# elfi-dev/elfi

Hardware: NVIDIA H100
Metric: accepted particles/sec (higher is better)
Workload: dtype f64

## Files before the change

### elfi_b200/csrc/common.cuh

```cuda
#pragma once

#include <cuda.h>
#include <cuda_runtime.h>

#include <cstdarg>
#include <cstdint>
#include <cstdio>
#include <cstring>

#include "../../include/elfi_b200.h"

namespace elfi {

void set_error(const char* fmt, ...);

#define ELFI_CUDA_OK(expr)                                                              \
    do {                                                                                \
        cudaError_t _e = (expr);                                                        \
        if (_e != cudaSuccess) {                                                        \
            ::elfi::set_error("%s failed: %s (%s:%d)", #expr, cudaGetErrorString(_e),   \
                              __FILE__, __LINE__);                                      \
            cudaGetLastError();       \
            return ELFI_B200_ERR_CUDA;                                                  \
        }                                                                               \
    } while (0)

#define ELFI_REQUIRE(cond, ...)                                                         \
    do {                                                                                \
        if (!(cond)) {                                                                  \
            ::elfi::set_error(__VA_ARGS__);                                             \
            return ELFI_B200_ERR_ARG;                                                   \
        }                                                                               \
    } while (0)

typedef CUresult (*tensor_map_encode_fn)(CUtensorMap*, CUtensorMapDataType, cuuint32_t, void*,
                                         const cuuint64_t*, const cuuint64_t*,
                                         const cuuint32_t*, const cuuint32_t*,
                                         CUtensorMapInterleave, CUtensorMapSwizzle,
                                         CUtensorMapL2promotion, CUtensorMapFloatOOBfill);

}

struct elfi_b200_ctx {
    int device;
    int sm_count;
    size_t smem_optin;
    elfi::tensor_map_encode_fn encode_tiled;
    void* scratch;
    size_t scratch_bytes;
    void* pinned;
    size_t pinned_bytes;
    void* dev_stage;
    size_t dev_stage_bytes;
    cudaStream_t copy_stream[2];
    cudaEvent_t copy_event[4];
};

namespace elfi {

void* ctx_scratch(elfi_b200_ctx* ctx, size_t bytes);

int make_rowmajor_f64_map(elfi_b200_ctx* ctx, const double* base, int64_t rows, int64_t cols,
                          int64_t ld, int box_rows, CUtensorMap* out);

inline bool tma_compatible(const void* base, int64_t ld) {
    return (reinterpret_cast<uintptr_t>(base) % 16 == 0) && ((ld * 8) % 16 == 0);
}

__device__ __forceinline__ uint32_t smem_u32(const void* p) {
    return static_cast<uint32_t>(__cvta_generic_to_shared(p));
}

__device__ __forceinline__ void mbar_init(uint32_t bar, uint32_t count) {
    asm volatile("mbarrier.init.shared::cta.b64 [%0], %1;" ::"r"(bar), "r"(count) : "memory");
}

__device__ __forceinline__ void mbar_fence_init() {
    asm volatile("fence.mbarrier_init.release.cluster;" ::: "memory");
    asm volatile("fence.proxy.async.shared::cta;" ::: "memory");
}

__device__ __forceinline__ void mbar_arrive_expect_tx(uint32_t bar, uint32_t bytes) {
    asm volatile("mbarrier.arrive.expect_tx.shared::cta.b64 _, [%0], %1;" ::"r"(bar), "r"(bytes)
                 : "memory");
}

__device__ __forceinline__ bool mbar_try_wait(uint32_t bar, uint32_t parity) {
    uint32_t ok;
    asm volatile(
        "{\n"
        ".reg .pred p;\n"
        "mbarrier.try_wait.parity.shared::cta.b64 p, [%1], %2;\n"
        "selp.u32 %0, 1, 0, p;\n"
// ... 35 lines not shown
```

### elfi_b200/csrc/ctx.cu

```cuda
#include "common.cuh"

namespace elfi {

static thread_local char g_error[512] = "";

void set_error(const char* fmt, ...) {
    va_list ap;
    va_start(ap, fmt);
    vsnprintf(g_error, sizeof(g_error), fmt, ap);
    va_end(ap);
}

void* ctx_scratch(elfi_b200_ctx* ctx, size_t bytes) {
    if (bytes <= ctx->scratch_bytes) return ctx->scratch;
    size_t want = bytes + (bytes >> 2) + (1u << 20);
    want = (want + 255) & ~size_t(255);
    if (ctx->scratch) {
        if (cudaDeviceSynchronize() != cudaSuccess || cudaFree(ctx->scratch) != cudaSuccess) {
            set_error("scratch release failed: %s", cudaGetErrorString(cudaGetLastError()));
            ctx->scratch = nullptr;
            ctx->scratch_bytes = 0;
            return nullptr;
        }
        ctx->scratch = nullptr;
        ctx->scratch_bytes = 0;
    }
    void* p = nullptr;
    cudaError_t e = cudaMalloc(&p, want);
    if (e != cudaSuccess) {
        set_error("cudaMalloc(%zu) for scratch failed: %s", want, cudaGetErrorString(e));
        cudaGetLastError();
        return nullptr;
    }
    ctx->scratch = p;
    ctx->scratch_bytes = want;
    return p;
}

int make_rowmajor_f64_map(elfi_b200_ctx* ctx, const double* base, int64_t rows, int64_t cols,
                          int64_t ld, int box_rows, CUtensorMap* out) {
    ELFI_REQUIRE(ctx->encode_tiled != nullptr, "cuTensorMapEncodeTiled entry point unavailable");
    ELFI_REQUIRE(tma_compatible(base, ld), "matrix is not TMA compatible (16-byte base/stride)");
    cuuint64_t dims[2] = {static_cast<cuuint64_t>(cols), static_cast<cuuint64_t>(rows)};
    cuuint64_t strides[1] = {static_cast<cuuint64_t>(ld) * sizeof(double)};
    cuuint32_t box[2] = {16u, static_cast<cuuint32_t>(box_rows)};
    cuuint32_t estr[2] = {1u, 1u};
    CUresult r = ctx->encode_tiled(out, CU_TENSOR_MAP_DATA_TYPE_FLOAT64, 2,
                                   const_cast<double*>(base), dims, strides, box, estr,
                                   CU_TENSOR_MAP_INTERLEAVE_NONE, CU_TENSOR_MAP_SWIZZLE_128B,
                                   CU_TENSOR_MAP_L2_PROMOTION_L2_256B,
                                   CU_TENSOR_MAP_FLOAT_OOB_FILL_NONE);
    if (r != CUDA_SUCCESS) {
        set_error("cuTensorMapEncodeTiled failed with CUresult %d (rows=%lld cols=%lld ld=%lld)",
                  static_cast<int>(r), (long long)rows, (long long)cols, (long long)ld);
        return ELFI_B200_ERR_CUDA;
    }
    return ELFI_B200_OK;
}

}

extern "C" {

int elfi_b200_version(void) { return ELFI_B200_VERSION; }

const char* elfi_b200_last_error(void) { return elfi::g_error; }

int elfi_b200_ctx_create(int device, elfi_b200_ctx** out) {
    ELFI_REQUIRE(out != nullptr, "ctx_create: out is NULL");
// ... 9 lines not shown
        elfi::set_error("ctx_create: device %d is sm_%d%d; this library is built for sm_90a only",
                        device, prop.major, prop.minor);
        return ELFI_B200_ERR_UNSUPPORTED;
    }
    elfi_b200_ctx* ctx = new elfi_b200_ctx();
    memset(ctx, 0, sizeof(*ctx));
    ctx->device = device;
    ctx->sm_count = prop.multiProcessorCount;
    ctx->smem_optin = prop.sharedMemPerBlockOptin;
    void* fn = nullptr;
    cudaDriverEntryPointQueryResult qres;
    cudaError_t e = cudaGetDriverEntryPoint("cuTensorMapEncodeTiled", &fn, cudaEnableDefault, &qres);
    if (e != cudaSuccess || qres != cudaDriverEntryPointSuccess || fn == nullptr) {
        elfi::set_error("ctx_create: cuTensorMapEncodeTiled not available from the driver");
        delete ctx;
        cudaGetLastError();
        return ELFI_B200_ERR_CUDA;
    }
    ctx->encode_tiled = reinterpret_cast<elfi::tensor_map_encode_fn>(fn);
    for (int i = 0; i < 2; ++i)
        ELFI_CUDA_OK(cudaStreamCreateWithFlags(&ctx->copy_stream[i], cudaStreamNonBlocking));
    for (int i = 0; i < 4; ++i)
        ELFI_CUDA_OK(cudaEventCreateWithFlags(&ctx->copy_event[i], cudaEventDisableTiming));
    *out = ctx;
    return ELFI_B200_OK;
}

int elfi_b200_ctx_destroy(elfi_b200_ctx* ctx) {
    if (!ctx) return ELFI_B200_OK;
    cudaSetDevice(ctx->device);
    cudaDeviceSynchronize();
    if (ctx->scratch) cudaFree(ctx->scratch);
    if (ctx->dev_stage) cudaFree(ctx->dev_stage);
    if (ctx->pinned) cudaFreeHost(ctx->pinned);
    for (int i = 0; i < 2; ++i)
        if (ctx->copy_stream[i]) cudaStreamDestroy(ctx->copy_stream[i]);
    for (int i = 0; i < 4; ++i)
        if (ctx->copy_event[i]) cudaEventDestroy(ctx->copy_event[i]);
    delete ctx;
    return ELFI_B200_OK;
}

int elfi_b200_ctx_sm_count(const elfi_b200_ctx* ctx) { return ctx ? ctx->sm_count : 0; }

int elfi_b200_allgather_particles(elfi_b200_ctx* const* ctxs, int64_t n_ctx, const double* const* send,
                                  int64_t rows, int64_t width, double* const* recv,
                                  void* const* streams) {
    ELFI_REQUIRE(ctxs && send && recv && streams && n_ctx >= 1 && n_ctx <= 64,
                 "allgather_particles: bad argument");
    ELFI_REQUIRE(rows >= 0 && width >= 1, "allgather_particles: bad shape");
    for (int64_t g = 0; g < n_ctx; ++g)
        ELFI_REQUIRE(ctxs[g] && (rows == 0 || (send[g] && recv[g])), "allgather_particles: NULL entry %lld",
                     (long long)g);
    if (rows == 0) return ELFI_B200_OK;
    const size_t bytes = size_t(rows) * size_t(width) * 8;
    int caller_device = 0;
    ELFI_CUDA_OK(cudaGetDevice(&caller_device));
    struct Restore {
        int d;
        ~Restore() { cudaSetDevice(d); }
    } restore{caller_device};
    for (int64_t d = 0; d < n_ctx; ++d) {
        ELFI_CUDA_OK(cudaSetDevice(ctxs[d]->device));
        for (int64_t s = 0; s < n_ctx; ++s) {
            if (ctxs[s]->device == ctxs[d]->device) continue;
            int can = 0;
// ... 34 lines not shown
```

### elfi_b200/csrc/distance.cu

```cuda
#include <cstdlib>

#include "rowstream.cuh"

extern "C" int elfi_b200_colmoments_f64(elfi_b200_ctx* ctx, const double* S, int64_t ldS, int64_t B,
                                        int64_t D, double* out, void* stream);

namespace elfi {

struct DistParams {
    const double* obs;
    const double* W;
    double* d_out;
    uint32_t* mask;
    int K;
    int has_thr;
    const double* shift_src;
    double* mom_partial;
    const double* thr_dev;
    double thr[ELFI_B200_MAX_NESTED];
    __device__ __forceinline__ double threshold(int k) const {
        return thr_dev ? __ldg(thr_dev + k) : thr[k];
    }
};

__device__ __forceinline__ void dist_setup_shared(uint8_t* aux, const DistParams& p, int D,
                                                  bool weighted) {
    const int Dp = ((D + RS_BOX_COLS - 1) / RS_BOX_COLS) * RS_BOX_COLS;
    double* obs_s = reinterpret_cast<double*>(aux);
    for (int j = threadIdx.x; j < Dp; j += blockDim.x) obs_s[j] = j < D ? p.obs[j] : 0.0;
    if (weighted) {
        double* w_s = obs_s + Dp;
        for (int k = 0; k < p.K; ++k)
            for (int j = threadIdx.x; j < Dp; j += blockDim.x)
                w_s[size_t(k) * Dp + j] = j < D ? p.W[size_t(k) * D + j] : 0.0;
// ... 273 lines not shown
dist_direct_kernel(const double* __restrict__ S, int64_t ld, int64_t B, int D, DistParams p) {
    const int64_t row = int64_t(blockIdx.x) * blockDim.x + threadIdx.x;
    const int lane = threadIdx.x & 31;
    const int K = p.K;
    bool ok = row < B;
    if (ok) {
        const double* r = S + row * ld;
        for (int k = 0; k < K; ++k) {
            double acc = 0.0;
            if (p.W != nullptr) {
                const double* w = p.W + size_t(k) * D;
                for (int j = 0; j < D; ++j) {
                    const double d = __dsub_rn(__ldg(r + j), __ldg(p.obs + j));
                    acc = __dadd_rn(acc, __dmul_rn(__ldg(w + j), __dmul_rn(d, d)));
                }
            } else {
                for (int j = 0; j < D; ++j) {
                    const double d = __dsub_rn(__ldg(r + j), __ldg(p.obs + j));
                    acc = __dadd_rn(acc, __dmul_rn(d, d));
                }
            }
            const double dist = sqrt(acc);
            p.d_out[row * K + k] = dist;
            if (p.has_thr) ok = ok && (dist <= p.threshold(k));
        }
    }
    if (p.mask != nullptr) {
        const uint32_t bits = __ballot_sync(0xffffffffu, ok && p.has_thr);
        if (lane == 0 && (row - lane) < B) p.mask[row >> 5] = bits;
    }
}

__global__ void __launch_bounds__(1024)
compact_mask_kernel(const uint32_t* __restrict__ mask, int64_t nwords, int64_t B,
                    int32_t* __restrict__ idx, int64_t* __restrict__ n_out) {
    __shared__ int64_t warp_sums[32];
    __shared__ int64_t base_s;
    const int tid = threadIdx.x;
    const int lane = tid & 31;
    const int wid = tid >> 5;
    const int64_t first = int64_t(blockIdx.x) * 1024;

    int64_t before = 0;
    for (int64_t w = tid; w < first; w += 1024) before += __popc(mask[w]);
    for (int o = 16; o > 0; o >>= 1) before += __shfl_xor_sync(0xffffffffu, before, o);
    if (lane == 0) warp_sums[wid] = before;
    __syncthreads();
    if (tid == 0) {
        int64_t t = 0;
        for (int i = 0; i < 32; ++i) t += warp_sums[i];
        base_s = t;
    }
    __syncthreads();
    const int64_t base = base_s;
    __syncthreads();

    const int64_t w = first + tid;
    const uint32_t bits = w < nwords ? mask[w] : 0u;
    const int cnt = __popc(bits);
    int incl = cnt;
    for (int o = 1; o < 32; o <<= 1) {
        const int t = __shfl_up_sync(0xffffffffu, incl, o);
        if (lane >= o) incl += t;
    }
    if (lane == 31) warp_sums[wid] = incl;
    __syncthreads();
    if (wid == 0) {
        int64_t v = warp_sums[lane];
        int64_t inc2 = v;
        for (int o = 1; o < 32; o <<= 1) {
            const int64_t t = __shfl_up_sync(0xffffffffu, inc2, o);
            if (lane >= o) inc2 += t;
        }
        warp_sums[lane] = inc2 - v;
        if (lane == 31 && blockIdx.x == gridDim.x - 1 && n_out != nullptr) *n_out = base + inc2;
    }
    __syncthreads();
    int64_t pos = base + warp_sums[wid] + (incl - cnt);
    if (idx != nullptr) {
        uint32_t b = bits;
        while (b) {
            const int bit = __ffs(b) - 1;
            b &= b - 1;
            idx[pos++] = int32_t(w * 32 + bit);
        }
    }
}

int launch_compact_mask(const uint32_t* mask, int64_t B, int32_t* idx, int64_t* n_out,
                        cudaStream_t stream) {
    const int64_t nwords = (B + 31) / 32;
    if (nwords == 0) {
        if (n_out) ELFI_CUDA_OK(cudaMemsetAsync(n_out, 0, sizeof(int64_t), stream));
        return ELFI_B200_OK;
    }
    const unsigned blocks = unsigned((nwords + 1023) / 1024);
    compact_mask_kernel<<<blocks, 1024, 0, stream>>>(mask, nwords, B, idx, n_out);
    ELFI_CUDA_OK(cudaGetLastError());
    return ELFI_B200_OK;
}

int launch_dist(elfi_b200_ctx* ctx, const double* S, int64_t ldS, int64_t B, int64_t D,
                const double* obs, const double* W, int64_t K, const double* thr_host,
                double* d_out, uint32_t* mask, cudaStream_t stream,
                const double* thr_dev = nullptr) {
    DistParams p;
    memset(&p, 0, sizeof(p));
    p.obs = obs;
    p.W = W;
    p.d_out = d_out;
    p.mask = mask;
    p.K = int(K);
    p.has_thr = thr_host != nullptr || thr_dev != nullptr;
    p.thr_dev = thr_dev;
    if (thr_host)
        for (int k = 0; k < K; ++k) p.thr[k] = thr_host[k];
    if (B == 0) return ELFI_B200_OK;

    const int64_t Dp = ((D + RS_BOX_COLS - 1) / RS_BOX_COLS) * RS_BOX_COLS;
    const bool use_tma = D >= RS_BOX_COLS && tma_compatible(S, ldS);
    if (use_tma) {
        const size_t aux = size_t(Dp) * 8 * (W ? (1 + K) : 1);
        if (rs_pick_stages(ctx->smem_optin, aux) >= 2) {
            if (W == nullptr) return rowstream_launch<EuclidConsumer>(ctx, S, ldS, B, D, aux, p, stream);
            if (K == 1) return rowstream_launch<WeightedConsumer>(ctx, S, ldS, B, D, aux, p, stream);
            if (K <= 2) return rowstream_launch<NestedConsumer<2>>(ctx, S, ldS, B, D, aux, p, stream);
            if (K <= 3) return rowstream_launch<NestedConsumer<3>>(ctx, S, ldS, B, D, aux, p, stream);
            if (K <= 4) return rowstream_launch<NestedConsumer<4>>(ctx, S, ldS, B, D, aux, p, stream);
            if (K <= 5) return rowstream_launch<NestedConsumer<5>>(ctx, S, ldS, B, D, aux, p, stream);
            if (K <= 6) return rowstream_launch<NestedConsumer<6>>(ctx, S, ldS, B, D, aux, p, stream);
// ... 224 lines not shown
    MetricParams p;
    memset(&p, 0, sizeof(p));
    p.obs = obs;
    p.V = V;
    p.d_out = d_out;
    p.mask = mask;
    p.K = 1;
    p.has_thr = thr_host != nullptr;
    if (thr_host) p.thr[0] = thr_host[0];
    if (B == 0) return ELFI_B200_OK;
    const int64_t Dp = ((D + RS_BOX_COLS - 1) / RS_BOX_COLS) * RS_BOX_COLS;
    const size_t aux = size_t(Dp) * 8 * 2;
    if (D >= RS_BOX_COLS && tma_compatible(S, ldS) && rs_pick_stages(ctx->smem_optin, aux) >= 2)
        return rowstream_launch<SeuclidConsumer>(ctx, S, ldS, B, D, aux, p, stream);
    seuclid_direct_kernel<<<unsigned((B + 255) / 256), 256, 0, stream>>>(S, ldS, B, int(D), p);
    ELFI_CUDA_OK(cudaGetLastError());
    return ELFI_B200_OK;
}

static int check_dist_args(const void* S, int64_t ldS, int64_t B, int64_t D, const void* obs,
                           const void* W, int64_t K, const void* thr, const void* acc_idx) {
    ELFI_REQUIRE(B >= 0 && D >= 1, "dist: bad shape B=%lld D=%lld", (long long)B, (long long)D);
    ELFI_REQUIRE(B == 0 || S != nullptr, "dist: S is NULL");
    ELFI_REQUIRE(obs != nullptr, "dist: obs is NULL");
    ELFI_REQUIRE(ldS >= D, "dist: ldS (%lld) < D (%lld)", (long long)ldS, (long long)D);
    ELFI_REQUIRE(K >= 1 && K <= ELFI_B200_MAX_NESTED, "dist: K=%lld outside [1, %d]",
                 (long long)K, ELFI_B200_MAX_NESTED);
    ELFI_REQUIRE(W != nullptr || K == 1, "dist: K=%lld needs a weight matrix", (long long)K);
    ELFI_REQUIRE(acc_idx == nullptr || thr != nullptr, "dist: acc_idx requires thresholds");
    ELFI_REQUIRE(B < (int64_t(1) << 31), "dist: B must fit int32 row indices");
    return ELFI_B200_OK;
}

}

extern "C" {

int elfi_b200_dist_euclid_thr_f64(elfi_b200_ctx* ctx, const double* S, int64_t ldS, int64_t B,
                                  int64_t D, const double* obs, const double* W, int64_t K,
                                  const double* thr_host, double* d_out, int32_t* acc_idx,
                                  int64_t* n_acc, void* stream_) {
    using namespace elfi;
    ELFI_REQUIRE(ctx != nullptr, "dist: ctx is NULL");
    int rc = check_dist_args(S, ldS, B, D, obs, W, K, thr_host, acc_idx);
    if (rc) return rc;
    ELFI_REQUIRE(B == 0 || d_out != nullptr, "dist: d_out is NULL");
    cudaStream_t stream = static_cast<cudaStream_t>(stream_);
    ELFI_CUDA_OK(cudaSetDevice(ctx->device));
    uint32_t* mask = nullptr;
    if (thr_host != nullptr) {
        const size_t nwords = size_t((B + 31) / 32);
        mask = static_cast<uint32_t*>(ctx_scratch(ctx, nwords * 4 + 256));
        if (!mask) return ELFI_B200_ERR_NOMEM;
    }
    rc = launch_dist(ctx, S, ldS, B, D, obs, W, K, thr_host, d_out, mask, stream);
    if (rc) return rc;
    if (thr_host != nullptr && (acc_idx != nullptr || n_acc != nullptr))
        return launch_compact_mask(mask, B, acc_idx, n_acc, stream);
    return ELFI_B200_OK;
}

int elfi_b200_dist_euclid_thr_dev_f64(elfi_b200_ctx* ctx, const double* S, int64_t ldS, int64_t B,
                                      int64_t D, const double* obs, const double* W, int64_t K,
                                      const double* thr_dev, double* d_out, int32_t* acc_idx,
                                      int64_t* n_acc, void* stream_) {
    using namespace elfi;
    ELFI_REQUIRE(ctx != nullptr && thr_dev != nullptr, "dist: ctx or thr_dev is NULL");
    int rc = check_dist_args(S, ldS, B, D, obs, W, K, thr_dev, acc_idx);
    if (rc) return rc;
    ELFI_REQUIRE(B == 0 || d_out != nullptr, "dist: d_out is NULL");
    cudaStream_t stream = static_cast<cudaStream_t>(stream_);
    ELFI_CUDA_OK(cudaSetDevice(ctx->device));
    const size_t nwords = size_t((B + 31) / 32);
    uint32_t* mask = static_cast<uint32_t*>(ctx_scratch(ctx, nwords * 4 + 256));
    if (!mask) return ELFI_B200_ERR_NOMEM;
    rc = launch_dist(ctx, S, ldS, B, D, obs, W, K, nullptr, d_out, mask, stream, thr_dev);
    if (rc) return rc;
    if (acc_idx != nullptr || n_acc != nullptr)
        return launch_compact_mask(mask, B, acc_idx, n_acc, stream);
    return ELFI_B200_OK;
}

int elfi_b200_dist_euclid_mom_f64(elfi_b200_ctx* ctx, const double* S, int64_t ldS, int64_t B,
                                  int64_t D, const double* obs, const double* W, int64_t K,
                                  const double* thr_host, const double* thr_dev, double* d_out,
                                  int32_t* acc_idx, int64_t* n_acc, double* moments,
                                  void* stream_) {
    using namespace elfi;
    ELFI_REQUIRE(ctx != nullptr && moments != nullptr, "dist_mom: ctx or moments is NULL");
    ELFI_REQUIRE(!(thr_host && thr_dev), "dist_mom: give thresholds on the host OR on the device");
    const void* thr = thr_host ? static_cast<const void*>(thr_host) : thr_dev;
    int rc = check_dist_args(S, ldS, B, D, obs, W, K, thr, acc_idx);
    if (rc) return rc;
    ELFI_REQUIRE(B >= 1 && d_out != nullptr, "dist_mom: needs at least one row and d_out");
    cudaStream_t stream = static_cast<cudaStream_t>(stream_);
    ELFI_CUDA_OK(cudaSetDevice(ctx->device));
    const int64_t Dp = ((D + RS_BOX_COLS - 1) / RS_BOX_COLS) * RS_BOX_COLS;
    const size_t aux = NestedMomentsConsumer<2>::aux_bytes(Dp, K);
    const bool fused = W != nullptr && D >= RS_BOX_COLS && tma_compatible(S, ldS) &&
                       rs_pick_stages(ctx->smem_optin, aux) >= 2;
    const size_t mask_bytes = (size_t((B + 31) / 32) * 4 + 255) & ~size_t(255);
    const size_t part_bytes = fused ? size_t(ctx->sm_count) * 16 * 2 * D * 8 : 0;
    uint8_t* base = static_cast<uint8_t*>(ctx_scratch(ctx, mask_bytes + part_bytes + 256));
    if (!base) return ELFI_B200_ERR_NOMEM;
    uint32_t* mask = thr ? reinterpret_cast<uint32_t*>(base) : nullptr;
    if (!fused) {
        rc = launch_dist(ctx, S, ldS, B, D, obs, W, K, thr_host, d_out, mask, stream, thr_dev);
        if (rc) return rc;
        if (thr && (acc_idx != nullptr || n_acc != nullptr)) {
// ... 172 lines not shown
```

### elfi_b200/csrc/select.cu

```cuda
#include <cstdlib>

#include "bitonic.cuh"
#include "eqweight.h"
#include "pairwise.cuh"

namespace elfi {

constexpr int SORT_CHUNK = 1024;
constexpr int SORT_WARPS = 8;

__global__ void __launch_bounds__(256)
sort_prepare_kernel(const double* __restrict__ keys, int64_t n, uint64_t* __restrict__ ukeys,
                    int32_t* __restrict__ vals, uint32_t* __restrict__ ghist) {
    __shared__ uint32_t h[8 * 256];
    for (int i = threadIdx.x; i < 8 * 256; i += blockDim.x) h[i] = 0;
    __syncthreads();
    const int64_t stride = int64_t(gridDim.x) * blockDim.x;
    for (int64_t i = int64_t(blockIdx.x) * blockDim.x + threadIdx.x; i < n; i += stride) {
        const uint64_t u = key_to_u64(keys[i]);
        ukeys[i] = u;
        vals[i] = int32_t(i);
#pragma unroll
        for (int p = 0; p < 8; ++p) atomicAdd(&h[p * 256 + ((u >> (8 * p)) & 255)], 1u);
    }
    __syncthreads();
    for (int i = threadIdx.x; i < 8 * 256; i += blockDim.x)
        if (h[i]) atomicAdd(&ghist[i], h[i]);
}

__device__ __forceinline__ bool pass_trivial(const uint32_t* ghist, int pass, int64_t n,
                                             uint64_t first_key) {
    return ghist[pass * 256 + ((first_key >> (8 * pass)) & 255)] == uint32_t(n);
}

__global__ void __launch_bounds__(SORT_WARPS * 32)
// ... 171 lines not shown
    int32_t col0[APPEND_MAX_SRC];
    int32_t n_src, total_width;
};

__global__ void __launch_bounds__(256)
accept_append_kernel(const int32_t* __restrict__ acc_idx, const int64_t* __restrict__ n_acc,
                     AppendSources src, double* __restrict__ dst, int64_t ld_dst, int64_t capacity,
                     const int64_t* __restrict__ count) {
    const int64_t base = *count;
    int64_t room = capacity - base;
    if (room < 0) room = 0;
    const int64_t rows = *n_acc < room ? *n_acc : room;
    const int64_t total = rows * src.total_width;
    const int64_t stride = int64_t(gridDim.x) * blockDim.x;
    for (int64_t t = int64_t(blockIdx.x) * blockDim.x + threadIdx.x; t < total; t += stride) {
        const int64_t j = t / src.total_width;
        const int c = int(t - j * src.total_width);
        const int64_t row = acc_idx ? int64_t(acc_idx[j]) : j;
        int k = 0;
#pragma unroll
        for (int q = 1; q < APPEND_MAX_SRC; ++q)
            if (q < src.n_src && c >= src.col0[q]) k = q;
        dst[(base + j) * ld_dst + c] = src.ptr[k][row * src.ld[k] + (c - src.col0[k])];
    }
}

__global__ void accept_count_kernel(const int64_t* __restrict__ n_acc, int64_t capacity,
                                    int64_t* __restrict__ count, int64_t* __restrict__ dropped) {
    int64_t room = capacity - *count;
    if (room < 0) room = 0;
    const int64_t rows = *n_acc < room ? *n_acc : room;
    if (dropped) *dropped += *n_acc - rows;
    *count += rows;
}

__global__ void __launch_bounds__(256)
gather2_rows_kernel(const double* __restrict__ A, int64_t ldA, int64_t nA,
                    const double* __restrict__ Bm, int64_t ldB, const int32_t* __restrict__ mapB,
                    const int32_t* __restrict__ perm, int64_t n, int64_t width,
                    double* __restrict__ dst, int64_t ld_dst) {
    const int64_t total = n * width;
    const int64_t stride = int64_t(gridDim.x) * blockDim.x;
    for (int64_t t = int64_t(blockIdx.x) * blockDim.x + threadIdx.x; t < total; t += stride) {
        const int64_t i = t / width, j = t - i * width;
        const int64_t r = perm ? perm[i] : i;
        double v;
        if (r < nA) {
            v = A[r * ldA + j];
        } else {
            const int64_t rb = mapB ? int64_t(mapB[r - nA]) : (r - nA);
            v = Bm[rb * ldB + j];
        }
        dst[i * ld_dst + j] = v;
    }
}

__global__ void __launch_bounds__(256)
merge_keys_kernel(const double* __restrict__ keysA, int64_t ldA, int64_t nA,
                  const double* __restrict__ keysB, int64_t ldB, const int32_t* __restrict__ mapB,
                  int64_t nB, double* __restrict__ out) {
    const int64_t stride = int64_t(gridDim.x) * blockDim.x;
    for (int64_t i = int64_t(blockIdx.x) * blockDim.x + threadIdx.x; i < nA + nB; i += stride) {
        if (i < nA) {
            out[i] = keysA[i * ldA];
        } else {
            const int64_t rb = mapB ? int64_t(mapB[i - nA]) : (i - nA);
// ... 296 lines not shown
        double incl = v;
        for (int o = 1; o < 32; o <<= 1) {
            const double t = __shfl_up_sync(0xffffffffu, incl, o);
            if (lane >= o) incl += t;
        }
        if (lane == 31) ws[wid] = incl;
        __syncthreads();
        double woff = 0.0;
        for (int q = 0; q < wid; ++q) woff += ws[q];
        const double carry = carry_s;
        const double c = (carry + woff + incl) / total;
        if (i < n - 1) {
            l0 += (c < alpha - eps) ? 1 : 0;
            l1 += (c < alpha + eps) ? 1 : 0;
        }
        __syncthreads();
        if (tid == 1023) carry_s = carry + woff + incl;
        __syncthreads();
    }
    for (int o = 16; o > 0; o >>= 1) {
        l0 += __shfl_xor_sync(0xffffffffu, l0, o);
        l1 += __shfl_xor_sync(0xffffffffu, l1, o);
    }
    if (lane == 0) { atomicAdd(&c0_s, l0); atomicAdd(&c1_s, l1); }
    __syncthreads();
    if (tid == 0) { atomicAdd(&counts[0], c0_s); atomicAdd(&counts[1], c1_s); }
}

__global__ void wq_pick_kernel(const uint64_t* __restrict__ ukeys, int64_t idx, double* __restrict__ out) {
    out[0] = u64_to_key(ukeys[idx]);
    out[1] = double(idx);
}

}

extern "C" {

int elfi_b200_sort_pairs_f64(elfi_b200_ctx* ctx, const double* keys, int64_t n,
                             double* keys_sorted, int32_t* perm, void* stream_) {
    using namespace elfi;
    ELFI_REQUIRE(ctx != nullptr, "sort: ctx is NULL");
    ELFI_REQUIRE(n >= 0 && n < (int64_t(1) << 31), "sort: n=%lld out of range", (long long)n);
    if (n == 0) return ELFI_B200_OK;
    ELFI_REQUIRE(keys != nullptr, "sort: keys is NULL");
    cudaStream_t stream = static_cast<cudaStream_t>(stream_);
    ELFI_CUDA_OK(cudaSetDevice(ctx->device));
    uint8_t* base = static_cast<uint8_t*>(ctx_scratch(ctx, sort_scratch_bytes(n)));
    if (!base) return ELFI_B200_ERR_NOMEM;
    SortScratch s = carve_sort(base, n);
    int rc = sort_pairs_device(keys, n, s, ctx->sm_count, stream);
    if (rc) return rc;
    int blocks = int((n + 255) / 256);
    if (blocks > ctx->sm_count * 8) blocks = ctx->sm_count * 8;
    sort_finish_kernel<<<blocks, 256, 0, stream>>>(s.k[0], s.v[0], n, keys_sorted, perm);
    ELFI_CUDA_OK(cudaGetLastError());
    return ELFI_B200_OK;
}

int elfi_b200_gather_rows_f64(elfi_b200_ctx* ctx, const double* src, int64_t ld_src,
                              const int32_t* idx, int64_t n, int64_t width, double* dst,
                              int64_t ld_dst, void* stream_) {
    using namespace elfi;
    ELFI_REQUIRE(ctx != nullptr, "gather: ctx is NULL");
    ELFI_REQUIRE(n >= 0 && width >= 1 && ld_src >= width && ld_dst >= width, "gather: bad shape");
    if (n == 0) return ELFI_B200_OK;
    ELFI_REQUIRE(src && idx && dst, "gather: NULL argument");
// ... 52 lines not shown
    int blocks = int((n + 255) / 256);
    if (blocks > ctx->sm_count * 8) blocks = ctx->sm_count * 8;
    merge_keys_kernel<<<blocks, 256, 0, stream>>>(keysA, ld_keysA, nA, keysB, ld_keysB, mapB, nB, keys);
    int rc = sort_pairs_device(keys, n, s, ctx->sm_count, stream);
    if (rc) return rc;
    const int32_t* perm = s.v[0];
    for (int64_t k = 0; k < n_out; ++k) {
        const int64_t width = width_host[k];
        ELFI_REQUIRE(width >= 1 && dst_host[k] && ld_dst_host[k] >= width &&
                     (nA == 0 || (A_host[k] && ldA_host[k] >= width)) &&
                     (nB == 0 || (B_host[k] && ldB_host[k] >= width)),
                     "topn_merge: bad descriptor of output %lld", (long long)k);
        int64_t gb = (n_keep * width + 255) / 256;
        if (gb > int64_t(ctx->sm_count) * 16) gb = int64_t(ctx->sm_count) * 16;
        gather2_rows_kernel<<<unsigned(gb), 256, 0, stream>>>(A_host[k], ldA_host[k], nA, B_host[k],
                                                              ldB_host[k], mapB, perm, n_keep, width,
                                                              dst_host[k], ld_dst_host[k]);
    }
    ELFI_CUDA_OK(cudaGetLastError());
    return ELFI_B200_OK;
}

int elfi_b200_accept_append_f64(elfi_b200_ctx* ctx, const int32_t* acc_idx, const int64_t* n_acc,
                                int64_t max_rows, int64_t n_src, const double* const* src_host,
                                const int64_t* ld_src_host, const int64_t* width_host, double* dst,
                                int64_t ld_dst, int64_t capacity, int64_t* count, int64_t* dropped,
                                void* stream_) {
    using namespace elfi;
    ELFI_REQUIRE(ctx && n_acc && src_host && ld_src_host && width_host && dst && count,
                 "accept_append: NULL argument");
    ELFI_REQUIRE(n_src >= 1 && n_src <= APPEND_MAX_SRC, "accept_append: 1..%d sources", APPEND_MAX_SRC);
    ELFI_REQUIRE(max_rows >= 0 && capacity >= 0, "accept_append: bad shape");
    AppendSources src;
    memset(&src, 0, sizeof(src));
    src.n_src = int32_t(n_src);
    int64_t col = 0;
    for (int k = 0; k < n_src; ++k) {
        ELFI_REQUIRE(src_host[k] && width_host[k] >= 1 && ld_src_host[k] >= width_host[k],
                     "accept_append: bad source %d", k);
        src.ptr[k] = src_host[k];
        src.ld[k] = ld_src_host[k];
        src.width[k] = int32_t(width_host[k]);
        src.col0[k] = int32_t(col);
        col += width_host[k];
    }
    ELFI_REQUIRE(col <= ld_dst && col < (int64_t(1) << 30), "accept_append: ld_dst < total width");
    src.total_width = int32_t(col);
    if (max_rows == 0) return ELFI_B200_OK;
    cudaStream_t stream = static_cast<cudaStream_t>(stream_);
    ELFI_CUDA_OK(cudaSetDevice(ctx->device));
    int64_t blocks = (max_rows * col + 255) / 256;
    if (blocks > int64_t(ctx->sm_count) * 8) blocks = int64_t(ctx->sm_count) * 8;
    accept_append_kernel<<<unsigned(blocks), 256, 0, stream>>>(acc_idx, n_acc, src, dst, ld_dst,
                                                              capacity, count);
    accept_count_kernel<<<1, 1, 0, stream>>>(n_acc, capacity, count, dropped);
    ELFI_CUDA_OK(cudaGetLastError());
    return ELFI_B200_OK;
}

extern "C" int elfi_b200_dist_euclid_thr_f64(elfi_b200_ctx*, const double*, int64_t, int64_t, int64_t,
                                             const double*, const double*, int64_t, const double*,
                                             double*, int32_t*, int64_t*, void*);
extern "C" int elfi_b200_dist_euclid_thr_dev_f64(elfi_b200_ctx*, const double*, int64_t, int64_t,
                                                 int64_t, const double*, const double*, int64_t,
                                                 const double*, double*, int32_t*, int64_t*, void*);

int elfi_b200_rejection_batch_f64(elfi_b200_ctx* ctx, const double* S, int64_t ldS, int64_t B,
                                  int64_t D, const double* obs, const double* W, int64_t K,
                                  const double* thr_host, const double* thr_dev, double* d_out,
                                  int32_t* acc_idx, int64_t* n_acc, int64_t n_extra,
                                  const double* const* extra_host, const int64_t* ld_extra_host,
                                  const int64_t* width_extra_host, double* dst, int64_t ld_dst,
                                  int64_t capacity, int64_t* count, int64_t* dropped,
                                  void* stream_) {
    using namespace elfi;
    ELFI_REQUIRE(ctx && acc_idx && n_acc && d_out, "rejection_batch: NULL argument");
    ELFI_REQUIRE((thr_host != nullptr) != (thr_dev != nullptr),
                 "rejection_batch: thresholds on the host OR on the device");
    ELFI_REQUIRE(n_extra >= 0 && n_extra < APPEND_MAX_SRC, "rejection_batch: 0..%d extra sources",
                 APPEND_MAX_SRC - 1);
    int rc = thr_host
        ? elfi_b200_dist_euclid_thr_f64(ctx, S, ldS, B, D, obs, W, K, thr_host, d_out, acc_idx, n_acc,
                                        stream_)
        : elfi_b200_dist_euclid_thr_dev_f64(ctx, S, ldS, B, D, obs, W, K, thr_dev, d_out, acc_idx,
                                            n_acc, stream_);
    if (rc) return rc;
    const double* src[APPEND_MAX_SRC];
    int64_t ld[APPEND_MAX_SRC], width[APPEND_MAX_SRC];
    src[0] = d_out; ld[0] = K; width[0] = K;
    for (int64_t k = 0; k < n_extra; ++k) {
        src[k + 1] = extra_host[k];
        ld[k + 1] = ld_extra_host[k];
        width[k + 1] = width_extra_host[k];
    }
    return elfi_b200_accept_append_f64(ctx, acc_idx, n_acc, B, n_extra + 1, src, ld, width, dst,
                                       ld_dst, capacity, count, dropped, stream_);
}

int elfi_b200_wquantile_f64(elfi_b200_ctx* ctx, const double* x, const double* w, int64_t n,
                            double alpha, double* out, void* stream_) {
    using namespace elfi;
    ELFI_REQUIRE(ctx != nullptr && x != nullptr && out != nullptr, "wquantile: NULL argument");
    ELFI_REQUIRE(n >= 1 && n < (int64_t(1) << 31), "wquantile: n=%lld out of range", (long long)n);
    ELFI_REQUIRE(alpha >= 0.0 && alpha <= 1.0, "wquantile: alpha=%g outside [0, 1]", alpha);
    cudaStream_t stream = static_cast<cudaStream_t>(stream_);
    ELFI_CUDA_OK(cudaSetDevice(ctx->device));
    const size_t sort_bytes = sort_scratch_bytes(n);
    const size_t extra = align256(size_t(n + 2) * 8) + 256;
    uint8_t* base = static_cast<uint8_t*>(ctx_scratch(ctx, sort_bytes + extra));
    if (!base) return ELFI_B200_ERR_NOMEM;
    SortScratch s = carve_sort(base, n);
    double* ws = reinterpret_cast<double*>(base + sort_bytes);
    double* total = reinterpret_cast<double*>(base + sort_bytes + align256(size_t(n) * 8));
    int rc = sort_pairs_device(x, n, s, ctx->sm_count, stream);
    if (rc) return rc;
    if (w == nullptr && alpha > 0.0) {
        wq_pick_kernel<<<1, 1, 0, stream>>>(s.k[0], equal_weight_cum_index(n, alpha) - 1, out);
        ELFI_CUDA_OK(cudaGetLastError());
        return ELFI_B200_OK;
    }
    if (alpha > 0.0 && n > 1) {
        const int64_t nb = (n + 4095) / 4096;
        double* partial = ws;
        int32_t* counts = reinterpret_cast<int32_t*>(total) + 4;
        const double eps = (4.0 * double(n) + 64.0) * 1.1102230246251565e-16;
        wq_par_block_sums_kernel<<<unsigned(nb), 1024, 0, stream>>>(w, s.v[0], n, partial);
        wq_par_scan_kernel<<<1, 1024, 0, stream>>>(partial, nb, counts);
        wq_par_count_kernel<<<unsigned(nb), 1024, 0, stream>>>(w, s.v[0], n, partial, nb, alpha, eps, counts);
        int32_t hc[2] = {0, -1};
// ... 52 lines not shown
```

Measured before the change: 24.80 million.

## Fuse mask compaction and accepted-row append into one kernel with ticket finalize

The rejection batch path now launches a single kernel that compacts the acceptance mask and gathers the accepted rows into the candidate buffer, replacing the separate compact and append launches. A global ticket counter lets the last block update count and dropped. The prefix popcount over earlier mask words is also vectorised with uint4 loads. This removes a kernel launch and the re-read of acc_idx and n_acc. The cost is a grid-wide atomic ticket and per-CTA redundant prefix work, plus new reliance on the ticket being reset correctly between calls.

Result: no change. 25.14 million (median of 6 runs) (+1.4%).

```diff
diff --git a/elfi_b200/csrc/common.cuh b/elfi_b200/csrc/common.cuh
--- a/elfi_b200/csrc/common.cuh
+++ b/elfi_b200/csrc/common.cuh
@@ -54,11 +54,14 @@
     size_t dev_stage_bytes;
     cudaStream_t copy_stream[2];
     cudaEvent_t copy_event[4];
+    unsigned int* ticket;
 };
 
 namespace elfi {
 
 void* ctx_scratch(elfi_b200_ctx* ctx, size_t bytes);
+
+unsigned int* ctx_ticket(elfi_b200_ctx* ctx);
 
 int make_rowmajor_f64_map(elfi_b200_ctx* ctx, const double* base, int64_t rows, int64_t cols,
                           int64_t ld, int box_rows, CUtensorMap* out);
diff --git a/elfi_b200/csrc/compact.cuh b/elfi_b200/csrc/compact.cuh
--- /dev/null
+++ b/elfi_b200/csrc/compact.cuh
@@ -0,0 +1,87 @@
+#pragma once
+
+#include "common.cuh"
+
+namespace elfi {
+
+__device__ __forceinline__ int64_t mask_prefix_popc(const uint32_t* __restrict__ mask, int64_t first,
+                                                    int64_t* warp_sums) {
+    const int tid = threadIdx.x, lane = tid & 31, wid = tid >> 5;
+    int64_t before = 0;
+    if ((reinterpret_cast<uintptr_t>(mask) & 15) == 0) {
+        const uint4* m4 = reinterpret_cast<const uint4*>(mask);
+        const int64_t n4 = first >> 2;
+        int64_t w = tid;
+        for (; w + 3 * 1024 < n4; w += 4 * 1024) {
+            uint4 v[4];
+#pragma unroll
+            for (int u = 0; u < 4; ++u) v[u] = m4[w + u * 1024];
+#pragma unroll
+            for (int u = 0; u < 4; ++u)
+                before += __popc(v[u].x) + __popc(v[u].y) + __popc(v[u].z) + __popc(v[u].w);
+        }
+        for (; w < n4; w += 1024) {
+            const uint4 v = m4[w];
+            before += __popc(v.x) + __popc(v.y) + __popc(v.z) + __popc(v.w);
+        }
+    } else {
+        for (int64_t w = tid; w < first; w += 1024) before += __popc(mask[w]);
+    }
+    for (int o = 16; o > 0; o >>= 1) before += __shfl_xor_sync(0xffffffffu, before, o);
+    if (lane == 0) warp_sums[wid] = before;
+    __syncthreads();
+    int64_t t = 0;
+    for (int i = 0; i < 32; ++i) t += warp_sums[i];
+    __syncthreads();
+    return t;
+}
+
+__device__ __forceinline__ int64_t compact_mask_block(const uint32_t* __restrict__ mask, int64_t nwords,
+                                                      int32_t* __restrict__ idx,
+                                                      int64_t* __restrict__ n_out, int* cta_count) {
+    __shared__ int64_t warp_sums[32];
+    __shared__ int cta_total;
+    const int tid = threadIdx.x;
+    const int lane = tid & 31;
+    const int wid = tid >> 5;
+    const int64_t first = int64_t(blockIdx.x) * 1024;
+    const int64_t base = mask_prefix_popc(mask, first, warp_sums);
+
+    const int64_t w = first + tid;
+    const uint32_t bits = w < nwords ? mask[w] : 0u;
+    const int cnt = __popc(bits);
+    int incl = cnt;
+    for (int o = 1; o < 32; o <<= 1) {
+        const int t = __shfl_up_sync(0xffffffffu, incl, o);
+        if (lane >= o) incl += t;
+    }
+    if (lane == 31) warp_sums[wid] = incl;
+    __syncthreads();
+    if (wid == 0) {
+        int64_t v = warp_sums[lane];
+        int64_t inc2 = v;
+        for (int o = 1; o < 32; o <<= 1) {
+            const int64_t t = __shfl_up_sync(0xffffffffu, inc2, o);
+            if (lane >= o) inc2 += t;
+        }
+        warp_sums[lane] = inc2 - v;
+        if (lane == 31) {
+            cta_total = int(inc2);
+            if (blockIdx.x == gridDim.x - 1 && n_out != nullptr) *n_out = base + inc2;
+        }
+    }
+    __syncthreads();
+    int64_t pos = base + warp_sums[wid] + (incl - cnt);
+    if (idx != nullptr) {
+        uint32_t b = bits;
+        while (b) {
+            const int bit = __ffs(b) - 1;
+            b &= b - 1;
+            idx[pos++] = int32_t(w * 32 + bit);
+        }
+    }
+    *cta_count = cta_total;
+    return base;
+}
+
+}
diff --git a/elfi_b200/csrc/ctx.cu b/elfi_b200/csrc/ctx.cu
--- a/elfi_b200/csrc/ctx.cu
+++ b/elfi_b200/csrc/ctx.cu
@@ -35,6 +35,21 @@
     ctx->scratch = p;
     ctx->scratch_bytes = want;
     return p;
+}
+
+unsigned int* ctx_ticket(elfi_b200_ctx* ctx) {
+    if (ctx->ticket) return ctx->ticket;
+    void* p = nullptr;
+    cudaError_t e = cudaMalloc(&p, 256);
+    if (e == cudaSuccess) e = cudaMemset(p, 0, 256);
+    if (e != cudaSuccess) {
+        set_error("ticket allocation failed: %s", cudaGetErrorString(e));
+        cudaGetLastError();
+        if (p) cudaFree(p);
+        return nullptr;
+    }
+    ctx->ticket = static_cast<unsigned int*>(p);
+    return ctx->ticket;
 }
 
 int make_rowmajor_f64_map(elfi_b200_ctx* ctx, const double* base, int64_t rows, int64_t cols,
@@ -110,6 +125,7 @@
     cudaDeviceSynchronize();
     if (ctx->scratch) cudaFree(ctx->scratch);
     if (ctx->dev_stage) cudaFree(ctx->dev_stage);
+    if (ctx->ticket) cudaFree(ctx->ticket);
     if (ctx->pinned) cudaFreeHost(ctx->pinned);
     for (int i = 0; i < 2; ++i)
         if (ctx->copy_stream[i]) cudaStreamDestroy(ctx->copy_stream[i]);
diff --git a/elfi_b200/csrc/distance.cu b/elfi_b200/csrc/distance.cu
--- a/elfi_b200/csrc/distance.cu
+++ b/elfi_b200/csrc/distance.cu
@@ -1,5 +1,6 @@
 #include <cstdlib>
 
+#include "compact.cuh"
 #include "rowstream.cuh"
 
 extern "C" int elfi_b200_colmoments_f64(elfi_b200_ctx* ctx, const double* S, int64_t ldS, int64_t B,
@@ -339,59 +340,10 @@
 }
 
 __global__ void __launch_bounds__(1024)
-compact_mask_kernel(const uint32_t* __restrict__ mask, int64_t nwords, int64_t B,
-                    int32_t* __restrict__ idx, int64_t* __restrict__ n_out) {
-    __shared__ int64_t warp_sums[32];
-    __shared__ int64_t base_s;
-    const int tid = threadIdx.x;
-    const int lane = tid & 31;
-    const int wid = tid >> 5;
-    const int64_t first = int64_t(blockIdx.x) * 1024;
-
-    int64_t before = 0;
-    for (int64_t w = tid; w < first; w += 1024) before += __popc(mask[w]);
-    for (int o = 16; o > 0; o >>= 1) before += __shfl_xor_sync(0xffffffffu, before, o);
-    if (lane == 0) warp_sums[wid] = before;
-    __syncthreads();
-    if (tid == 0) {
-        int64_t t = 0;
-        for (int i = 0; i < 32; ++i) t += warp_sums[i];
-        base_s = t;
-    }
-    __syncthreads();
-    const int64_t base = base_s;
-    __syncthreads();
-
-    const int64_t w = first + tid;
-    const uint32_t bits = w < nwords ? mask[w] : 0u;
-    const int cnt = __popc(bits);
-    int incl = cnt;
-    for (int o = 1; o < 32; o <<= 1) {
-        const int t = __shfl_up_sync(0xffffffffu, incl, o);
-        if (lane >= o) incl += t;
-    }
-    if (lane == 31) warp_sums[wid] = incl;
-    __syncthreads();
-    if (wid == 0) {
-        int64_t v = warp_sums[lane];
-        int64_t inc2 = v;
-        for (int o = 1; o < 32; o <<= 1) {
-            const int64_t t = __shfl_up_sync(0xffffffffu, inc2, o);
-            if (lane >= o) inc2 += t;
-        }
-        warp_sums[lane] = inc2 - v;
-        if (lane == 31 && blockIdx.x == gridDim.x - 1 && n_out != nullptr) *n_out = base + inc2;
-    }
-    __syncthreads();
-    int64_t pos = base + warp_sums[wid] + (incl - cnt);
-    if (idx != nullptr) {
-        uint32_t b = bits;
-        while (b) {
-            const int bit = __ffs(b) - 1;
-            b &= b - 1;
-            idx[pos++] = int32_t(w * 32 + bit);
-        }
-    }
+compact_mask_kernel(const uint32_t* __restrict__ mask, int64_t nwords, int32_t* __restrict__ idx,
+                    int64_t* __restrict__ n_out) {
+    int cta_count;
+    compact_mask_block(mask, nwords, idx, n_out, &cta_count);
 }
 
 int launch_compact_mask(const uint32_t* mask, int64_t B, int32_t* idx, int64_t* n_out,
@@ -402,7 +354,7 @@
         return ELFI_B200_OK;
     }
     const unsigned blocks = unsigned((nwords + 1023) / 1024);
-    compact_mask_kernel<<<blocks, 1024, 0, stream>>>(mask, nwords, B, idx, n_out);
+    compact_mask_kernel<<<blocks, 1024, 0, stream>>>(mask, nwords, idx, n_out);
     ELFI_CUDA_OK(cudaGetLastError());
     return ELFI_B200_OK;
 }
@@ -693,6 +645,25 @@
     return ELFI_B200_OK;
 }
 
+int dist_thr_launch(elfi_b200_ctx* ctx, const double* S, int64_t ldS, int64_t B, int64_t D,
+                    const double* obs, const double* W, int64_t K, const double* thr_host,
+                    const double* thr_dev, double* d_out, const int32_t* acc_idx, uint32_t** mask,
+                    cudaStream_t stream) {
+    ELFI_REQUIRE(ctx != nullptr, "dist: ctx is NULL");
+    const void* thr = thr_host ? static_cast<const void*>(thr_host) : thr_dev;
+    int rc = check_dist_args(S, ldS, B, D, obs, W, K, thr, acc_idx);
+    if (rc) return rc;
+    ELFI_REQUIRE(B == 0 || d_out != nullptr, "dist: d_out is NULL");
+    ELFI_CUDA_OK(cudaSetDevice(ctx->device));
+    *mask = nullptr;
+    if (thr != nullptr) {
+        const size_t nwords = size_t((B + 31) / 32);
+        *mask = static_cast<uint32_t*>(ctx_scratch(ctx, nwords * 4 + 256));
+        if (!*mask) return ELFI_B200_ERR_NOMEM;
+    }
+    return launch_dist(ctx, S, ldS, B, D, obs, W, K, thr_host, d_out, *mask, stream, thr_dev);
+}
+
 }
 
 extern "C" {
@@ -702,19 +673,10 @@
                                   const double* thr_host, double* d_out, int32_t* acc_idx,
                                   int64_t* n_acc, void* stream_) {
     using namespace elfi;
-    ELFI_REQUIRE(ctx != nullptr, "dist: ctx is NULL");
-    int rc = check_dist_args(S, ldS, B, D, obs, W, K, thr_host, acc_idx);
-    if (rc) return rc;
-    ELFI_REQUIRE(B == 0 || d_out != nullptr, "dist: d_out is NULL");
     cudaStream_t stream = static_cast<cudaStream_t>(stream_);
-    ELFI_CUDA_OK(cudaSetDevice(ctx->device));
     uint32_t* mask = nullptr;
-    if (thr_host != nullptr) {
-        const size_t nwords = size_t((B + 31) / 32);
-        mask = static_cast<uint32_t*>(ctx_scratch(ctx, nwords * 4 + 256));
-        if (!mask) return ELFI_B200_ERR_NOMEM;
-    }
-    rc = launch_dist(ctx, S, ldS, B, D, obs, W, K, thr_host, d_out, mask, stream);
+    int rc = dist_thr_launch(ctx, S, ldS, B, D, obs, W, K, thr_host, nullptr, d_out, acc_idx, &mask,
+                             stream);
     if (rc) return rc;
     if (thr_host != nullptr && (acc_idx != nullptr || n_acc != nullptr))
         return launch_compact_mask(mask, B, acc_idx, n_acc, stream);
@@ -726,16 +688,11 @@
                                       const double* thr_dev, double* d_out, int32_t* acc_idx,
                                       int64_t* n_acc, void* stream_) {
     using namespace elfi;
-    ELFI_REQUIRE(ctx != nullptr && thr_dev != nullptr, "dist: ctx or thr_dev is NULL");
-    int rc = check_dist_args(S, ldS, B, D, obs, W, K, thr_dev, acc_idx);
-    if (rc) return rc;
-    ELFI_REQUIRE(B == 0 || d_out != nullptr, "dist: d_out is NULL");
+    ELFI_REQUIRE(thr_dev != nullptr, "dist: thr_dev is NULL");
     cudaStream_t stream = static_cast<cudaStream_t>(stream_);
-    ELFI_CUDA_OK(cudaSetDevice(ctx->device));
-    const size_t nwords = size_t((B + 31) / 32);
-    uint32_t* mask = static_cast<uint32_t*>(ctx_scratch(ctx, nwords * 4 + 256));
-    if (!mask) return ELFI_B200_ERR_NOMEM;
-    rc = launch_dist(ctx, S, ldS, B, D, obs, W, K, nullptr, d_out, mask, stream, thr_dev);
+    uint32_t* mask = nullptr;
+    int rc = dist_thr_launch(ctx, S, ldS, B, D, obs, W, K, nullptr, thr_dev, d_out, acc_idx, &mask,
+                             stream);
     if (rc) return rc;
     if (acc_idx != nullptr || n_acc != nullptr)
         return launch_compact_mask(mask, B, acc_idx, n_acc, stream);
diff --git a/elfi_b200/csrc/select.cu b/elfi_b200/csrc/select.cu
--- a/elfi_b200/csrc/select.cu
+++ b/elfi_b200/csrc/select.cu
@@ -1,6 +1,7 @@
 #include <cstdlib>
 
 #include "bitonic.cuh"
+#include "compact.cuh"
 #include "eqweight.h"
 #include "pairwise.cuh"
 
@@ -238,6 +239,45 @@
     const int64_t rows = *n_acc < room ? *n_acc : room;
     if (dropped) *dropped += *n_acc - rows;
     *count += rows;
+}
+
+__global__ void __launch_bounds__(1024)
+compact_append_kernel(const uint32_t* __restrict__ mask, int64_t nwords, int32_t* acc_idx,
+                      int64_t* n_acc, AppendSources src, double* __restrict__ dst, int64_t ld_dst,
+                      int64_t capacity, int64_t* count, int64_t* dropped, unsigned int* ticket) {
+    __shared__ int64_t count0_s;
+    if (threadIdx.x == 0) count0_s = *count;
+    int cta_count;
+    const int64_t base = compact_mask_block(mask, nwords, acc_idx, n_acc, &cta_count);
+    __syncthreads();
+    const int64_t count0 = count0_s;
+    int64_t room = capacity - count0;
+    if (room < 0) room = 0;
+    const int64_t hi = base + cta_count < room ? base + cta_count : room;
+    const int64_t total = hi > base ? (hi - base) * src.total_width : 0;
+    for (int64_t t = threadIdx.x; t < total; t += blockDim.x) {
+        const int64_t j = base + t / src.total_width;
+        const int c = int(t % src.total_width);
+        const int64_t row = acc_idx[j];
+        int k = 0;
+#pragma unroll
+        for (int q = 1; q < APPEND_MAX_SRC; ++q)
+            if (q < src.n_src && c >= src.col0[q]) k = q;
+        dst[(count0 + j) * ld_dst + c] = src.ptr[k][row * src.ld[k] + (c - src.col0[k])];
+    }
+    if (blockIdx.x == gridDim.x - 1 && threadIdx.x == 31) __threadfence();
+    __syncthreads();
+    if (threadIdx.x == 0) {
+        const unsigned int t = atomicAdd(ticket, 1u);
+        if (t == gridDim.x - 1) {
+            __threadfence();
+            const int64_t n = *reinterpret_cast<volatile int64_t*>(n_acc);
+            const int64_t rows = n < room ? n : room;
+            if (dropped) *dropped += n - rows;
+            *count = count0 + rows;
+            *ticket = 0u;
+        }
+    }
 }
 
 __global__ void __launch_bounds__(256)
@@ -600,6 +640,30 @@
     out[1] = double(idx);
 }
 
+static int append_sources(int64_t n_src, const double* const* src_host, const int64_t* ld_src_host,
+                          const int64_t* width_host, int64_t ld_dst, AppendSources* src) {
+    memset(src, 0, sizeof(*src));
+    src->n_src = int32_t(n_src);
+    int64_t col = 0;
+    for (int k = 0; k < n_src; ++k) {
+        ELFI_REQUIRE(src_host[k] && width_host[k] >= 1 && ld_src_host[k] >= width_host[k],
+                     "accept_append: bad source %d", k);
+        src->ptr[k] = src_host[k];
+        src->ld[k] = ld_src_host[k];
+        src->width[k] = int32_t(width_host[k]);
+        src->col0[k] = int32_t(col);
+        col += width_host[k];
+    }
+    ELFI_REQUIRE(col <= ld_dst && col < (int64_t(1) << 30), "accept_append: ld_dst < total width");
+    src->total_width = int32_t(col);
+    return ELFI_B200_OK;
+}
+
+int dist_thr_launch(elfi_b200_ctx* ctx, const double* S, int64_t ldS, int64_t B, int64_t D,
+                    const double* obs, const double* W, int64_t K, const double* thr_host,
+                    const double* thr_dev, double* d_out, const int32_t* acc_idx, uint32_t** mask,
+                    cudaStream_t stream);
+
 }
 
 extern "C" {
@@ -718,24 +782,12 @@
     ELFI_REQUIRE(n_src >= 1 && n_src <= APPEND_MAX_SRC, "accept_append: 1..%d sources", APPEND_MAX_SRC);
     ELFI_REQUIRE(max_rows >= 0 && capacity >= 0, "accept_append: bad shape");
     AppendSources src;
-    memset(&src, 0, sizeof(src));
-    src.n_src = int32_t(n_src);
-    int64_t col = 0;
-    for (int k = 0; k < n_src; ++k) {
-        ELFI_REQUIRE(src_host[k] && width_host[k] >= 1 && ld_src_host[k] >= width_host[k],
-                     "accept_append: bad source %d", k);
-        src.ptr[k] = src_host[k];
-        src.ld[k] = ld_src_host[k];
-        src.width[k] = int32_t(width_host[k]);
-        src.col0[k] = int32_t(col);
-        col += width_host[k];
-    }
-    ELFI_REQUIRE(col <= ld_dst && col < (int64_t(1) << 30), "accept_append: ld_dst < total width");
-    src.total_width = int32_t(col);
+    int rc = append_sources(n_src, src_host, ld_src_host, width_host, ld_dst, &src);
+    if (rc) return rc;
     if (max_rows == 0) return ELFI_B200_OK;
     cudaStream_t stream = static_cast<cudaStream_t>(stream_);
     ELFI_CUDA_OK(cudaSetDevice(ctx->device));
-    int64_t blocks = (max_rows * col + 255) / 256;
+    int64_t blocks = (max_rows * src.total_width + 255) / 256;
     if (blocks > int64_t(ctx->sm_count) * 8) blocks = int64_t(ctx->sm_count) * 8;
     accept_append_kernel<<<unsigned(blocks), 256, 0, stream>>>(acc_idx, n_acc, src, dst, ld_dst,
                                                               capacity, count);
@@ -743,13 +795,6 @@
     ELFI_CUDA_OK(cudaGetLastError());
     return ELFI_B200_OK;
 }
-
-extern "C" int elfi_b200_dist_euclid_thr_f64(elfi_b200_ctx*, const double*, int64_t, int64_t, int64_t,
-                                             const double*, const double*, int64_t, const double*,
-                                             double*, int32_t*, int64_t*, void*);
-extern "C" int elfi_b200_dist_euclid_thr_dev_f64(elfi_b200_ctx*, const double*, int64_t, int64_t,
-                                                 int64_t, const double*, const double*, int64_t,
-                                                 const double*, double*, int32_t*, int64_t*, void*);
 
 int elfi_b200_rejection_batch_f64(elfi_b200_ctx* ctx, const double* S, int64_t ldS, int64_t B,
                                   int64_t D, const double* obs, const double* W, int64_t K,
@@ -765,22 +810,36 @@
                  "rejection_batch: thresholds on the host OR on the device");
     ELFI_REQUIRE(n_extra >= 0 && n_extra < APPEND_MAX_SRC, "rejection_batch: 0..%d extra sources",
                  APPEND_MAX_SRC - 1);
-    int rc = thr_host
-        ? elfi_b200_dist_euclid_thr_f64(ctx, S, ldS, B, D, obs, W, K, thr_host, d_out, acc_idx, n_acc,
-                                        stream_)
-        : elfi_b200_dist_euclid_thr_dev_f64(ctx, S, ldS, B, D, obs, W, K, thr_dev, d_out, acc_idx,
-                                            n_acc, stream_);
-    if (rc) return rc;
-    const double* src[APPEND_MAX_SRC];
+    ELFI_REQUIRE(dst && count && capacity >= 0, "rejection_batch: bad candidate buffer");
+    ELFI_REQUIRE(n_extra == 0 || (extra_host && ld_extra_host && width_extra_host),
+                 "rejection_batch: NULL extra source descriptor");
+    const double* srcs[APPEND_MAX_SRC];
     int64_t ld[APPEND_MAX_SRC], width[APPEND_MAX_SRC];
-    src[0] = d_out; ld[0] = K; width[0] = K;
+    srcs[0] = d_out; ld[0] = K; width[0] = K;
     for (int64_t k = 0; k < n_extra; ++k) {
-        src[k + 1] = extra_host[k];
+        srcs[k + 1] = extra_host[k];
         ld[k + 1] = ld_extra_host[k];
         width[k + 1] = width_extra_host[k];
     }
-    return elfi_b200_accept_append_f64(ctx, acc_idx, n_acc, B, n_extra + 1, src, ld, width, dst,
-                                       ld_dst, capacity, count, dropped, stream_);
+    AppendSources src;
+    int rc = append_sources(n_extra + 1, srcs, ld, width, ld_dst, &src);
+    if (rc) return rc;
+    cudaStream_t stream = static_cast<cudaStream_t>(stream_);
+    uint32_t* mask = nullptr;
+    rc = dist_thr_launch(ctx, S, ldS, B, D, obs, W, K, thr_host, thr_dev, d_out, acc_idx, &mask,
+                         stream);
+    if (rc) return rc;
+    const int64_t nwords = (B + 31) / 32;
+    if (nwords == 0) {
+        ELFI_CUDA_OK(cudaMemsetAsync(n_acc, 0, sizeof(int64_t), stream));
+        return ELFI_B200_OK;
+    }
+    unsigned int* ticket = ctx_ticket(ctx);
+    if (!ticket) return ELFI_B200_ERR_CUDA;
+    compact_append_kernel<<<unsigned((nwords + 1023) / 1024), 1024, 0, stream>>>(
+        mask, nwords, acc_idx, n_acc, src, dst, ld_dst, capacity, count, dropped, ticket);
+    ELFI_CUDA_OK(cudaGetLastError());
+    return ELFI_B200_OK;
 }
 
 int elfi_b200_wquantile_f64(elfi_b200_ctx* ctx, const double* x, const double* w, int64_t n,
```
